# thanh-nt25/Whisper-context-biasing

Hardware: AMD Instinct MI355X
Metric: audio-seconds/sec (RTF) + biased-WER, whisper-small 30s clips, batch32 (higher is better)
Workload: dtype bf16

## Files before the change

### whisper_context_biasing_amd/csrc/k_logmel.hip

```cpp
#include <type_traits>

#include "common.h"
#include "kernels.h"

namespace wcb {

constexpr int kNFFT = 400, kHop = 160, kFrames = 3000, kNSamp = 480000;
constexpr int kFPB = 64;
constexpr int kSpan = (kFPB - 1) * kHop + 416;
constexpr int kNCol = 416;
constexpr int kBins = 201;

WCB_DEV unsigned ord_enc(float f) {
  const unsigned u = __float_as_uint(f);
  return (u & 0x80000000u) ? ~u : (u | 0x80000000u);
}
WCB_DEV float ord_dec(unsigned u) { return __uint_as_float((u & 0x80000000u) ? (u & 0x7fffffffu) : ~u); }

struct MelFixed {};
struct MelLong { int n_total, T, T_ld; const int* n_valid; };
template <bool SPLIT, bool LONG = false>
__global__ __launch_bounds__(256) void logmel_power_mel_kernel(const float* __restrict__ pcm, long pcm_stride, int n_valid,
                                                               const float* __restrict__ dft, const uint16_t* __restrict__ dft3,
                                                               const int* __restrict__ mel_lo,
                                                               const int* __restrict__ mel_hi, const float* __restrict__ mel_w,
                                                               int n_mel, float* __restrict__ out, unsigned* __restrict__ clip_max,
                                                               [[maybe_unused]] std::conditional_t<LONG, MelLong, MelFixed> shape) {
  constexpr int kPowLd = kBins + 3;
  constexpr int kLdsFloats = (kSpan > kFPB * kPowLd) ? kSpan : kFPB * kPowLd;
  __shared__ __attribute__((aligned(16))) float lds[kLdsFloats];
  __shared__ float wmax[4];
  const int b = blockIdx.y, f0 = blockIdx.x * kFPB;
  const int tid = threadIdx.x, lane = tid & 63, wave = tid >> 6;
  const float* x = pcm + (long)b * pcm_stride;
  int nS = kNSamp, nF = kFrames, ldo = kFrames;
  if constexpr (LONG) { nS = shape.n_total; nF = shape.T; ldo = shape.T_ld; n_valid = shape.n_valid[b]; }
// ... 75 lines not shown
  }
  }
  __syncthreads();
#pragma unroll
  for (int i = 0; i < 4; ++i)
#pragma unroll
    for (int j = 0; j < kCW; ++j)
#pragma unroll
      for (int e = 0; e < 4; ++e) {
        const float v = acc[i][j][e];
        const float p = v * v + __shfl_xor(v, 1, 64) * __shfl_xor(v, 1, 64);
        const int col = (cf0 + j) * 16 + (lane & 15);
        if (j < ncf && (col & 1) == 0 && (col >> 1) < kBins)
          lds[(i * 16 + (lane >> 4) * 4 + e) * kPowLd + (col >> 1)] = p;
      }
  __syncthreads();
  float lmax = -INFINITY;
  for (int idx = tid; idx < n_mel * kFPB; idx += 256) {
    const int m = idx / kFPB, f = idx % kFPB;
    if (f0 + f >= nF) continue;
    const int lo = mel_lo[m], hi = mel_hi[m];
    float s = 0.f;
    for (int k = lo; k < hi; ++k) s = fmaf(mel_w[m * 32 + (k - lo)], lds[f * kPowLd + k], s);
    const float lg = log10f(fmaxf(s, 1e-10f));
    out[((long)b * n_mel + m) * ldo + f0 + f] = lg;
    lmax = fmaxf(lmax, lg);
  }
  lmax = wave_max(lmax);
  if (lane == 0) wmax[wave] = lmax;
  __syncthreads();
  if (tid == 0) atomicMax(clip_max + b, ord_enc(fmaxf(fmaxf(wmax[0], wmax[1]), fmaxf(wmax[2], wmax[3]))));
}

__global__ void logmel_normalize_kernel(float* mel, const unsigned* clip_max, int n_per_clip, long total) {
  for (long i = blockIdx.x * (long)blockDim.x + threadIdx.x; i < total; i += (long)gridDim.x * blockDim.x) {
    const float mx = ord_dec(clip_max[i / n_per_clip]);
    mel[i] = (fmaxf(mel[i], mx - 8.0f) + 4.0f) / 4.0f;
  }
}

__global__ void logmel_normalize_long_kernel(float* mel, const unsigned* clip_max, int n_mel, int T, int T_ld, long total) {
  for (long i = blockIdx.x * (long)blockDim.x + threadIdx.x; i < total; i += (long)gridDim.x * blockDim.x) {
    const long row = i / T;
    const float mx = ord_dec(clip_max[row / n_mel]);
    float* p = mel + row * T_ld + (i - row * T);
    *p = (fmaxf(*p, mx - 8.0f) + 4.0f) / 4.0f;
  }
}

void logmel_power_mel(const float* pcm, long pcm_stride, int n_samples, int B, const float* dft, const void* dft3,
                      const int* mel_lo, const int* mel_hi, const float* mel_w, int n_mel, float* mel_out,
                      unsigned* clip_max, hipStream_t s) {
  (void)hipMemsetAsync(clip_max, 0, sizeof(unsigned) * B, s);
  const dim3 grid((kFrames + kFPB - 1) / kFPB, B);
  if (dft3)
    WCB_LAUNCH(logmel_power_mel_kernel<true>, grid, dim3(256), 0, s, pcm, pcm_stride, n_samples, dft,
               reinterpret_cast<const uint16_t*>(dft3), mel_lo, mel_hi, mel_w, n_mel, mel_out, clip_max, MelFixed{});
  else
    WCB_LAUNCH(logmel_power_mel_kernel<false>, grid, dim3(256), 0, s, pcm, pcm_stride, n_samples, dft,
               nullptr, mel_lo, mel_hi, mel_w, n_mel, mel_out, clip_max, MelFixed{});
}

void logmel_long(const float* pcm, long pcm_stride, const int* n_valid, int n_total, int B, const float* dft, const void* dft3,
                 const int* mel_lo, const int* mel_hi, const float* mel_w, int n_mel, float* mel_out, int T_ld,
                 unsigned* clip_max, hipStream_t s) {
  const int T = n_total / kHop;
  (void)hipMemsetAsync(clip_max, 0, sizeof(unsigned) * B, s);
  const dim3 grid((T + kFPB - 1) / kFPB, B);
  const MelLong shape{n_total, T, T_ld, n_valid};
  if (dft3)
    WCB_LAUNCH((logmel_power_mel_kernel<true, true>), grid, dim3(256), 0, s, pcm, pcm_stride, 0, dft,
               reinterpret_cast<const uint16_t*>(dft3), mel_lo, mel_hi, mel_w, n_mel, mel_out, clip_max, shape);
  else
    WCB_LAUNCH((logmel_power_mel_kernel<false, true>), grid, dim3(256), 0, s, pcm, pcm_stride, 0, dft,
               nullptr, mel_lo, mel_hi, mel_w, n_mel, mel_out, clip_max, shape);
  const long total = (long)B * n_mel * T;
  WCB_LAUNCH(logmel_normalize_long_kernel, dim3(2048), dim3(256), 0, s, mel_out, clip_max, n_mel, T, T_ld, total);
}

void logmel_normalize(float* mel, const unsigned* clip_max, int B, int n_mel, hipStream_t s) {
  const long total = (long)B * n_mel * kFrames;
  WCB_LAUNCH(logmel_normalize_kernel, dim3(2048), dim3(256), 0, s, mel, clip_max, n_mel * kFrames, total);
}

template <typename T>
__global__ void mel_to_conv_input_kernel(const float* __restrict__ mel, int n_mel, T* __restrict__ xt, long clip_stride) {
  __shared__ float tile[64][65];
  const int b = blockIdx.z, t0 = blockIdx.x * 64, c0 = blockIdx.y * 64;
  for (int i = threadIdx.x; i < 64 * 64; i += 256) {
    const int c = c0 + i / 64, t = t0 + i % 64;
    tile[i / 64][i % 64] = (c < n_mel && t < kFrames) ? mel[((long)b * n_mel + c) * kFrames + t] : 0.f;
  }
  __syncthreads();
  for (int i = threadIdx.x; i < 64 * 64; i += 256) {
    const int t = t0 + i / 64, c = c0 + i % 64;
    if (t < kFrames && c < n_mel) xt[(long)b * clip_stride + (long)(t + 1) * n_mel + c] = DT<T>::fromf(tile[i % 64][i / 64]);
  }
  if (blockIdx.x == 0 && blockIdx.y == 0)
    for (int c = threadIdx.x; c < n_mel; c += 256) {
      xt[(long)b * clip_stride + c] = DT<T>::fromf(0.f);
      xt[(long)b * clip_stride + (long)(kFrames + 1) * n_mel + c] = DT<T>::fromf(0.f);
    }
}
// ... 46 lines not shown
```

### whisper_context_biasing_amd/csrc/kernels.h

```cpp
#pragma once
#include <hip/hip_runtime.h>
#include <hip/hip_ext.h>
#include <stdint.h>

#include "tsrule.h"

namespace wcb {

struct LaunchTimer {
  hipEvent_t start = nullptr, stop = nullptr;
  int n = 0;
  const void* fn = nullptr;
  long grid = 0;
};
inline thread_local LaunchTimer g_launch_timer;

#define WCB_LAUNCH(K, G, B, SH, S, ...)                                                              \
  do {                                                                                               \
    ::wcb::LaunchTimer& lt_ = ::wcb::g_launch_timer;                                                 \
    if (lt_.stop) {                                                                                  \
      if (!lt_.n) {                                                                                  \
        lt_.fn = reinterpret_cast<const void*>(K);                                                   \
        const dim3 g_ = dim3(G), b_ = dim3(B);                                                       \
        lt_.grid = (long)g_.x * g_.y * g_.z * b_.x * b_.y * b_.z;                                    \
// ... 97 lines not shown
  const int* phys = nullptr; long phys_ld = 0;
  int causal = 0;
  int q_log2 = 0;
  int xcd_nqb = 0;
  int kv_rows = 0;
  const int* key_start = nullptr;
};
void attention_decode(DType t, const AttnArgs& a, hipStream_t s);
bool attention_flash(DType t, const AttnArgs& a, hipStream_t s);

constexpr int kXencMaxSplit = 16;
struct XencArgs {
  const void* enc = nullptr; long enc_sb = 0;
  const void* qp = nullptr;
  int rows = 0, H = 0, D = 0, S = 0;
  int nsplit = 1;
  float* part = nullptr;
  float* ml = nullptr;
  Stamp stamp;
  int variant = 1;
  int row0 = 0, rows_per_enc = 1;
  int fm = 0;
  int part16 = 0;
  int merge_os = 1;
};
bool xenc_supported(DType t, int D);
void xenc_to_fm(DType t, const void* src, void* dst, int B, int S, int D, hipStream_t s);
long xenc_fm_elems(int B, int S, int D);
void xenc_attention(DType t, const XencArgs& a, hipStream_t s);
void xenc_merge(DType t, const XencArgs& a, void* u, long ldu, hipStream_t s);
void xenc_merge_v(DType t, const XencArgs& a, const void* wv, const float* bv, void* o, long ldo, hipStream_t s,
                  const void* wv_fm = nullptr);

void logmel_power_mel(const float* pcm, long pcm_stride, int n_samples, int B, const float* dft, const void* dft3,
                      const int* mel_lo, const int* mel_hi, const float* mel_w, int n_mel,
                      float* mel_out, unsigned* clip_max, hipStream_t s);
void logmel_normalize(float* mel, const unsigned* clip_max, int B, int n_mel, hipStream_t s);
void mel_to_conv_input(DType t, const float* mel, int B, int n_mel, void* xt, long clip_stride,
                       hipStream_t s);
void logmel_long(const float* pcm, long pcm_stride, const int* n_valid, int n_total, int B, const float* dft, const void* dft3,
                 const int* mel_lo, const int* mel_hi, const float* mel_w, int n_mel, float* mel_out, int T_ld,
                 unsigned* clip_max, hipStream_t s);
void mel_window_to_conv_input(DType t, const float* mel, int n_mel, int T_ld, const int* clip_idx, const int* seek, const int* nfr,
                              int rows, void* xt, long row_stride, hipStream_t s);

struct ForestArgs {
  const int* root = nullptr;
  const int* rc_off = nullptr;
  const int* rc_tok = nullptr;
  const int* rc_dst = nullptr;
};
void forest_init(const ForestArgs& f, int* state, int* rowbase, int R, int nb, hipStream_t s);

struct SelectArgs {
  const float* logits = nullptr; long ld = 0; int M = 0; int V = 0;
  float lam = 0.f; const uint32_t* root_bits = nullptr;
  const int* trans_off = nullptr; const int* trans_tok = nullptr; const int* trans_dst = nullptr;
  const int* root_child = nullptr;
  const int* st_depth = nullptr; const int* st_keep = nullptr;
  int* state = nullptr; int* finished = nullptr;
  int* rowbase = nullptr;
  int eos = 0, pad = 0; int min_new = 0;
  int* step = nullptr;
  int* pos = nullptr;
  int* next_ids = nullptr; int* out_ids = nullptr; int out_ld = 0;
  float* part_val = nullptr; int* part_idx = nullptr; int nchunk = 0;
  int* all_done = nullptr;
  unsigned long long* ticket_unfin = nullptr;
  float* out_score = nullptr;
  const float* part_max = nullptr; const float* part_sum = nullptr;
  float* out_logprob = nullptr;
  const void* emb = nullptr; const void* pemb = nullptr; int n_pos = 0, d = 0, dtype = 0;
  float* x = nullptr; void* x16 = nullptr; void* x16fm = nullptr; int fm_nw = 0, fm_kpw = 0;
// ... 134 lines not shown
```

### whisper_context_biasing_amd/csrc/runtime.cpp

```cpp
#include <hip/hip_runtime.h>

#include <algorithm>
#include <cxxabi.h>
#include <cmath>
#include <cstdio>
#include <cstring>
#include <map>
#include <thread>
#include <memory>
#include <stdexcept>
#include <string>
#include <vector>
#include <cstdlib>
#include <deque>
#include <atomic>

#include "../../include/wcb.h"
#include "kernels.h"
#include "sample.h"
#include "dtw.h"

using namespace wcb;

namespace {
// ... 165 lines not shown
};

struct wcb_handle {
  wcb_model_desc d{};
  DType dt = kBF16;
  int device = 0;
  std::string err;
  hipStream_t he = nullptr;
  static constexpr int kMaxCtx = 4;
  int nctx = 2;
  hipEvent_t ev_xkv[kMaxCtx] = {}, ev_dec[kMaxCtx] = {};
  int gen_count = 0;
  hipEvent_t ev_in = nullptr, ev_out = nullptr;
  static constexpr int kMaxSub = DecCtx::kMaxSub;
  DecCtx dc[kMaxCtx];
  int n_sub = 1;
  int xsplit = 1;
  int xvariant = 0;
  int flash_split = 2;
  int beam_xattn = 0;
  int ln_fold = 1;
  int merge_v = 1;
  int xpart16 = 1;
  int xq_kq = 0;
  int ring_kt = 2;
  int beam_wide = 1;
  int beam_wfm = 0;
  int lean_fold = 1;
  int xqk = 1;
  int xqk_nch = 8;
  int merge_os = 1;
  int lm_walkers = 256;
  int mel_split = 0;
  int lean_mf2 = 0;
  int beam_chunks = 0;
  int beam_raster = 0;
  int lm_ln_split = 0;
  int enc_flash_qw = 4;
  int xmode = 1;
  int beam_xmode = 0;
  int group_rows = 512;
  int xenc_split = 6;
  int xenc_fm = 1;
  int xenc_variant = 1;
  int ln16 = 1;
  int vocab_pad = 0;
  int steps_per_graph = 8;
  int lean = 1;
  int lean_x = 1;
  int64_t n_graph_captures = 0;
  struct wcb_state* step_state = nullptr;
  bool rules_on = false, rules_has0 = false;
  TsRule rules_ts;
  DevBuf rules_deny, rules_deny0;
  int enc_raster = 8;
  int enc_gemm = 4;
  bool dec_gemm = false;
  std::map<std::string, DevBuf> staged;
  std::vector<DevBuf> owned;
  bool ready = false;
  int dbg_enc_layers = -1;
  void *conv1_w = nullptr, *conv2_w = nullptr;
  float *conv1_b = nullptr, *conv2_b = nullptr, *enc_pos = nullptr;
  int k1pad = 0;
  std::vector<LayerW> enc, dec;
  float *enc_ln_w = nullptr, *enc_ln_b = nullptr, *dec_ln_w = nullptr, *dec_ln_b = nullptr;
  void* xkv_w = nullptr; float* xkv_b = nullptr;
  void *tok_emb = nullptr, *dec_pos = nullptr;
  void* tok_emb_fm = nullptr;
  DevBuf dft, dft3, mel_lo, mel_hi, mel_w, clip_max;
  DevBuf win_ints;
  int enc_B = 0;
  DevBuf xt, hbuf, x, h, qkv, att, ffn, encout;
  DevBuf xkv2[kMaxCtx];
  DevBuf al_w, al_M, al_tf, al_lens, al_frames, al_prefix, al_trace;
  int last_gen_buf = -1, last_gen_B = 0, last_gen_xm = 0, last_gen_id = -1;
  hipEvent_t ev_align = nullptr;
  bool align_pending = false;
  size_t align_ws_bytes = (size_t)1 << 30;
  std::unique_ptr<wcb_bias> empty_bias;
  std::vector<wcb_bias*> biases;
  DevBuf dev_err;
  bool prof = false, prof_stamps = false;
  std::vector<ProfEntry> prof_e;
  std::deque<std::pair<int, std::pair<hipEvent_t, hipEvent_t>>> prof_pending;
  std::vector<hipEvent_t> ev_pool;
  DevBuf stamps, stamp_acc;
  static constexpr int kStampRegions = 8;
  unsigned long long* stamp_base(int buf, int region) {
    return stamps.as<unsigned long long>() + ((size_t)buf * kStampRegions + region) * stamp_slots() * 2 * kStampSub;
  }
  double xattn_bytes = 0, xattn_flops = 0;
  long stamp_slots() const { return (long)d.n_text_ctx * d.n_layers * kMaxSub; }

  int H() const { return d.n_heads; }
  int S() const { return d.n_audio_ctx; }

  void* upload(const void* src, size_t bytes) {
    owned.emplace_back();
    owned.back().ensure(bytes);
    HIPCHK(hipMemcpy(owned.back().p, src, bytes, hipMemcpyHostToDevice));
    return owned.back().p;
  }
// ... 87 lines not shown
    f();
    return WCB_OK;
  } catch (const WcbError& e) {
    (h ? h->err : g_err) = e.what();
    return e.code;
  } catch (const std::exception& e) {
    (h ? h->err : g_err) = e.what();
    return WCB_ERR_ARG;
  }
}

double hz_to_mel(double f) { return f >= 1000.0 ? 15.0 + std::log(f / 1000.0) * (27.0 / std::log(6.4)) : 3.0 * f / 200.0; }
double mel_to_hz(double m) { return m >= 15.0 ? 1000.0 * std::exp((std::log(6.4) / 27.0) * (m - 15.0)) : 200.0 * m / 3.0; }

std::vector<double> mel_filters(int n_mel) {
  const int nf = 201;
  std::vector<double> mf(n_mel + 2), ff(n_mel + 2), fft(nf), out((size_t)nf * n_mel, 0.0);
  const double mmin = hz_to_mel(0.0), mmax = hz_to_mel(8000.0);
  for (int i = 0; i < n_mel + 2; ++i) {
    mf[i] = (i == n_mel + 1) ? mmax : mmin + i * ((mmax - mmin) / (n_mel + 1));
    ff[i] = mel_to_hz(mf[i]);
  }
  for (int k = 0; k < nf; ++k) fft[k] = (k == nf - 1) ? 8000.0 : k * (8000.0 / (nf - 1));
  for (int k = 0; k < nf; ++k)
    for (int m = 0; m < n_mel; ++m) {
      const double down = -(ff[m] - fft[k]) / (ff[m + 1] - ff[m]);
      const double up = (ff[m + 2] - fft[k]) / (ff[m + 2] - ff[m + 1]);
      const double v = std::max(0.0, std::min(down, up));
      out[(size_t)k * n_mel + m] = v * (2.0 / (ff[m + 2] - ff[m]));
    }
  return out;
}

}

extern "C" {

const char* wcb_last_error(const wcb_handle* h) { return h ? h->err.c_str() : g_err.c_str(); }

int wcb_create(const wcb_model_desc* desc, int device, wcb_handle** out) {
  return guarded(nullptr, [&] {
    REQUIRE(desc && out, "null argument");
    REQUIRE(desc->d_model % 64 == 0 && desc->d_model / desc->n_heads == 64, "head_dim must be 64");
    REQUIRE(desc->dtype >= 0 && desc->dtype <= 2, "dtype");
    REQUIRE(desc->n_mel == 80 || desc->n_mel == 128, "n_mel must be 80 or 128");
    REQUIRE(desc->n_audio_ctx * 2 == kFrames, "n_audio_ctx must be 1500");
    HIPCHK(hipSetDevice(device));
    auto h = std::make_unique<wcb_handle>();
    h->d = *desc;
    h->dt = DType(desc->dtype);
    h->device = device;
    HIPCHK(hipStreamCreateWithPriority(&h->he, hipStreamNonBlocking, 0));
    for (int ci = 0; ci < wcb_handle::kMaxCtx; ++ci) {
      DecCtx& D = h->dc[ci];
      HIPCHK(hipEventCreateWithFlags(&D.ev_fork, hipEventDisableTiming));
      HIPCHK(hipHostMalloc(reinterpret_cast<void**>(&D.done_h), 2 * sizeof(int), hipHostMallocDefault));
      for (hipEvent_t& e : D.ev_poll) HIPCHK(hipEventCreateWithFlags(&e, hipEventDisableTiming));
      for (int i = 0; i < DecCtx::kMaxSub; ++i) HIPCHK(hipEventCreateWithFlags(&D.ev_join[i], hipEventDisableTiming));
    }
    for (int i = 0; i < wcb_handle::kMaxCtx; ++i) {
      HIPCHK(hipEventCreateWithFlags(&h->ev_xkv[i], hipEventDisableTiming));
      HIPCHK(hipEventCreateWithFlags(&h->ev_dec[i], hipEventDisableTiming));
    }
    HIPCHK(hipEventCreateWithFlags(&h->ev_in, hipEventDisableTiming));
    HIPCHK(hipEventCreateWithFlags(&h->ev_out, hipEventDisableTiming));
    h->xvariant = desc->n_heads >= 20 ? 1 : 0;
    h->xmode = xenc_supported(h->dt, desc->d_model) ? 1 : 0;
    h->beam_xmode = 0;
    if (h->dt == kF32) h->ln16 = 0;
    h->dec_gemm = gemm_dec_supported(h->dt, desc->d_model);
    std::vector<float> dft((size_t)kNCol * kNCol, 0.f);
    for (int c = 0; c < 402; ++c) {
      const int bin = c >> 1;
      for (int k = 0; k < 400; ++k) {
        const double win = 0.5 - 0.5 * std::cos(2.0 * M_PI * k / 400.0);
        const double ang = 2.0 * M_PI * (double)((long)bin * k % 400) / 400.0;
        dft[(size_t)c * kNCol + k] = (float)(win * ((c & 1) ? -std::sin(ang) : std::cos(ang)));
      }
    }
    h->dft.ensure(dft.size() * 4);
    HIPCHK(hipMemcpy(h->dft.p, dft.data(), dft.size() * 4, hipMemcpyHostToDevice));
    {
      auto bf = [](double v, double& back) -> uint16_t {
        const float f = (float)v;
        uint32_t u;
        std::memcpy(&u, &f, 4);
        u += 0x7fffu + ((u >> 16) & 1u);
        const uint16_t hbits = (uint16_t)(u >> 16);
        const uint32_t w = (uint32_t)hbits << 16;
        float g;
        std::memcpy(&g, &w, 4);
        back = g;
        return hbits;
      };
      std::vector<uint16_t> t3((size_t)3 * kNCol * kNCol, 0);
      for (int c = 0; c < 402; ++c) {
        const int bin = c >> 1;
        for (int k = 0; k < 400; ++k) {
          const double win = 0.5 - 0.5 * std::cos(2.0 * M_PI * k / 400.0);
          const double ang = 2.0 * M_PI * (double)((long)bin * k % 400) / 400.0;
          double r = win * ((c & 1) ? -std::sin(ang) : std::cos(ang)), back;
          for (int part = 0; part < 3; ++part) {
            t3[(size_t)part * kNCol * kNCol + (size_t)c * kNCol + k] = bf(r, back);
            r -= back;
          }
        }
      }
      h->dft3.ensure(t3.size() * 2);
      HIPCHK(hipMemcpy(h->dft3.p, t3.data(), t3.size() * 2, hipMemcpyHostToDevice));
    }
    const auto fb = mel_filters(desc->n_mel);
    std::vector<int> lo(desc->n_mel), hi(desc->n_mel);
    std::vector<float> w((size_t)desc->n_mel * 32, 0.f);
    for (int m = 0; m < desc->n_mel; ++m) {
      int a = -1, b = -1;
      for (int k = 0; k < 201; ++k)
        if ((float)fb[(size_t)k * desc->n_mel + m] != 0.f) { if (a < 0) a = k; b = k; }
      if (a < 0) { a = 0; b = -1; }
      REQUIRE(b - a + 1 <= 32, "mel filter wider than 32 bins");
      lo[m] = a;
      hi[m] = b + 1;
      for (int k = a; k <= b; ++k) w[(size_t)m * 32 + (k - a)] = (float)fb[(size_t)k * desc->n_mel + m];
    }
    h->mel_lo.ensure(lo.size() * 4);
    h->mel_hi.ensure(hi.size() * 4);
    h->mel_w.ensure(w.size() * 4);
    HIPCHK(hipMemcpy(h->mel_lo.p, lo.data(), lo.size() * 4, hipMemcpyHostToDevice));
    HIPCHK(hipMemcpy(h->mel_hi.p, hi.data(), hi.size() * 4, hipMemcpyHostToDevice));
    HIPCHK(hipMemcpy(h->mel_w.p, w.data(), w.size() * 4, hipMemcpyHostToDevice));
    auto eb = std::make_unique<wcb_bias>();
    eb->vocab = desc->vocab;
    const int nw = (desc->vocab + 31) / 32;
    eb->root_bits.ensure((size_t)nw * 4);
    eb->root_child.ensure((size_t)desc->vocab * 4);
    HIPCHK(hipMemsetAsync(eb->root_child.p, 0xff, (size_t)desc->vocab * 4, nullptr));
    HIPCHK(hipStreamSynchronize(nullptr));
    std::vector<int> off = {0, 0};
    eb->trans_off.ensure(8);
    HIPCHK(hipMemcpy(eb->trans_off.p, off.data(), 8, hipMemcpyHostToDevice));
    eb->trans_tok.ensure(4);
    eb->trans_dst.ensure(4);
    eb->st_depth.ensure(4);
// ... 4 lines not shown
  });
}

void wcb_destroy(wcb_handle* h) {
  if (!h) return;
  (void)hipSetDevice(h->device);
  (void)hipDeviceSynchronize();
  for (wcb_bias* b : h->biases) b->owner = nullptr;
  for (DecCtx& D : h->dc) {
    D.drop_graphs();
    for (DevBuf* b : {&D.kvself, &D.dx, &D.dx16, &D.dx16fm, &D.dh, &D.dq, &D.dqp, &D.du, &D.datt, &D.dffn, &D.dstats, &D.drst, &D.xpart, &D.xml, &D.xticket,
                      &D.logits, &D.part_val, &D.part_idx, &D.ints, &D.outbuf, &D.forced, &D.beam, &D.kq_cnt, &D.part_max, &D.part_sum,
                      &D.lpbuf})
      b->release();
    if (D.ev_fork) (void)hipEventDestroy(D.ev_fork);
    for (hipEvent_t e : D.ev_poll)
      if (e) (void)hipEventDestroy(e);
    if (D.done_h) (void)hipHostFree(D.done_h);
    D.forest.release();
    D.poff.release();
    D.nsp.release();
    D.lang.release();
    if (D.p_stage) (void)hipHostFree(D.p_stage);
    if (D.ev_pcopy) (void)hipEventDestroy(D.ev_pcopy);
    if (D.f_stage) (void)hipHostFree(D.f_stage);
    if (D.ev_fcopy) (void)hipEventDestroy(D.ev_fcopy);
    for (int i = 0; i < DecCtx::kMaxSub; ++i) {
      if (D.ev_join[i]) (void)hipEventDestroy(D.ev_join[i]);
      if (D.sub[i]) (void)hipStreamDestroy(D.sub[i]);
    }
    if (D.hs) (void)hipStreamDestroy(D.hs);
  }
  for (auto& b : h->owned) b.release();
  for (DevBuf* b : {&h->dft, &h->dft3, &h->mel_lo, &h->mel_hi, &h->mel_w, &h->clip_max, &h->win_ints, &h->xt, &h->hbuf, &h->x, &h->h,
                    &h->qkv, &h->att, &h->ffn, &h->encout, &h->stamps, &h->stamp_acc, &h->dev_err, &h->rules_deny,
                    &h->rules_deny0, &h->al_w, &h->al_M, &h->al_tf, &h->al_lens, &h->al_frames, &h->al_prefix, &h->al_trace})
    b->release();
  for (auto e : h->ev_pool) (void)hipEventDestroy(e);
  if (h->ev_align) (void)hipEventDestroy(h->ev_align);
  if (h->ev_in) (void)hipEventDestroy(h->ev_in);
  if (h->ev_out) (void)hipEventDestroy(h->ev_out);
  if (h->he) (void)hipStreamDestroy(h->he);
  for (int i = 0; i < wcb_handle::kMaxCtx; ++i) {
    h->xkv2[i].release();
    if (h->ev_xkv[i]) (void)hipEventDestroy(h->ev_xkv[i]);
    if (h->ev_dec[i]) (void)hipEventDestroy(h->ev_dec[i]);
  }
  delete h;
}

namespace {
void quiesce(wcb_handle* h);
void drop_graphs(wcb_handle* h);
}

int wcb_set_option(wcb_handle* h, const char* name, int value) {
  return guarded(h, [&] {
    REQUIRE(h && name, "bad argument");
    const std::string n = name;
    static const char* const kFreeWhileStepwise[] = {"decode_contexts", "enc_flash", "enc_gemm", "enc_raster",
                                                     "steps_per_graph", "kq_cnt_seed", "align_ws"};
    bool free_opt = false;
    for (const char* f : kFreeWhileStepwise) free_opt |= n == f;
    REQUIRE(free_opt || !h->step_state, "option " + n + ": a step-wise decode is active (wcb_decode_end first)");
    if (n == "xmode" || n == "beam_xmode") {
      REQUIRE(!h->ready, "option " + n + " selects the weight layouts: set it before wcb_finalize_weights");
      REQUIRE(value == 0 || value == 1, "option " + n + ": 0 or 1");
// ... 33 lines not shown
      }
    } else if (n == "align_ws") {
      REQUIRE(value >= 1 && value <= 65536, "option align_ws: 1..65536 (MiB)");
      h->align_ws_bytes = (size_t)value << 20;
    } else if (n == "steps_per_graph") {
      REQUIRE(value >= 1 && value <= 64, "option steps_per_graph: 1..64");
      h->steps_per_graph = value;
    } else if (n == "xenc_fm") {
      h->xenc_fm = value != 0;
    } else if (n == "xq_kq") {
      h->xq_kq = value != 0;
    } else if (n == "enc_gemm") {
      REQUIRE(value == 0 || value == 1 || value == 4 || value == 5, "option enc_gemm: 0, 1, 4 or 5");
      h->enc_gemm = value;
    } else if (n == "enc_raster") {
      REQUIRE(value >= 0 && value <= 64, "option enc_raster: 0..64");
      h->enc_raster = value;
    } else if (n == "lean") {
      REQUIRE(!h->ready, "option lean selects weight layouts: set it before wcb_finalize_weights");
      h->lean = value != 0;
    } else if (n == "lean_x") {
      h->lean_x = value != 0;
    } else if (n == "xpart16") {
      h->xpart16 = value != 0;
    } else if (n == "merge_v") {
      h->merge_v = value != 0;
    } else if (n == "ln_fold") {
      REQUIRE(!h->ready, "option ln_fold selects weight layouts: set it before wcb_finalize_weights");
      h->ln_fold = value != 0;
    } else if (n == "lean_mf2") {
      h->lean_mf2 = value != 0;
    } else if (n == "mel_split") {
      h->mel_split = value != 0;
    } else if (n == "lm_walkers") {
      REQUIRE(!h->ready, "option lm_walkers sizes the argmax partials: set it before wcb_finalize_weights");
      REQUIRE(value == 128 || value == 192 || value == 256 || value == 384 || value == 512 || value == 1024,
              "option lm_walkers: 128, 192, 256, 384, 512 or 1024");
      h->lm_walkers = value;
    } else if (n == "merge_os") {
      REQUIRE(value == 1 || value == 2, "option merge_os: 1 or 2");
      h->merge_os = value;
    } else if (n == "xqk_chunks") {
      REQUIRE(value == 2 || value == 4 || value == 8 || value == 16, "option xqk_chunks: 2, 4, 8 or 16");
      h->xqk_nch = value;
    } else if (n == "xqk") {
      h->xqk = value != 0;
    } else if (n == "lean_fold") {
      REQUIRE(!h->ready, "option lean_fold selects weight layouts: set it before wcb_finalize_weights");
      h->lean_fold = value != 0;
    } else if (n == "beam_chunks") {
      h->beam_chunks = value != 0;
    } else if (n == "beam_wfm") {
      REQUIRE(!h->ready, "option beam_wfm selects weight layouts: set it before wcb_finalize_weights");
      h->beam_wfm = value != 0;
    } else if (n == "beam_raster") {
      REQUIRE(value >= 0 && value <= 64, "option beam_raster: 0..64");
      h->beam_raster = value;
    } else if (n == "beam_wide") {
      REQUIRE(!h->ready, "option beam_wide selects weight layouts: set it before wcb_finalize_weights");
      h->beam_wide = value != 0;
    } else if (n == "beam_xattn") {
      REQUIRE(value >= 0 && value <= 3, "option beam_xattn: 0..3");
      h->beam_xattn = value;
    } else if (n == "flash_split") {
      REQUIRE(value >= 1 && value <= kXSplit, "option flash_split: 1..8");
      h->flash_split = value;
// ... 1218 lines not shown
  }
  g.key = key;
}

struct GenCall {
  const float* mel; int B; const wcb_gen_cfg* cfg;
  const int32_t* prefix; int prefix_len;
  int32_t *out_ids, *out_steps;
  void* stream;
  const wcb_bias* bias = nullptr; const wcb_bias_batch* bb = nullptr;
  float *out_logprobs = nullptr, *out_seq_scores = nullptr;
  const wcb_sample_cfg* smp = nullptr;
  const int32_t* prompts = nullptr; int prompt_ld = 0; const int32_t* prompt_len = nullptr;
  const wcb_windows* win = nullptr; float* out_no_speech = nullptr;
  const wcb_lang_cfg* lang = nullptr;
};

DecCtx& step_ctx(wcb_handle* h, const wcb_state* st, bool what = true, const char* msg = "bad argument (state of this handle)") {
  REQUIRE(h && st && st->h == h && h->step_state == st && what, msg);
  return h->dc[wcb_handle::kMaxCtx - 1];
}

}

extern "C" {

int wcb_log_mel(wcb_handle* h, const float* pcm, int B, int n_samples, int64_t pcm_stride, float* mel_out, void* stream) {
  return guarded(h, [&] {
    REQUIRE(h && pcm && mel_out && B > 0 && n_samples > 0, "bad argument");
    REQUIRE(pcm_stride >= std::min(n_samples, kNSamp), "pcm_stride < n_samples");
    if ((size_t)B * 4 > h->clip_max.bytes) { quiesce(h); h->clip_max.ensure((size_t)std::max(B, h->enc_B) * 4); }
    sync_in(h, stream, h->he);
    h->timed("log_mel", 0, (double)B * (std::min(n_samples, kNSamp) * 4.0 + h->d.n_mel * kFrames * 4.0 * 3), h->he, [&] {
      logmel_power_mel(pcm, (long)pcm_stride, n_samples, B, h->dft.as<float>(), h->mel_split ? h->dft3.p : nullptr,
                       h->mel_lo.as<int>(), h->mel_hi.as<int>(),
                       h->mel_w.as<float>(), h->d.n_mel, mel_out, h->clip_max.as<unsigned>(), h->he);
      logmel_normalize(mel_out, h->clip_max.as<unsigned>(), B, h->d.n_mel, h->he);
    });
    sync_out(h, stream, h->he);
  });
}

int wcb_encode(wcb_handle* h, const float* mel, int B, void* enc_out, void* stream) {
  return guarded(h, [&] {
    REQUIRE(h && mel && B > 0, "bad argument");
    if (!h->ready) throw WcbError(WCB_ERR_STATE, "weights not finalized");
    ensure_enc_ws(h, B);
    sync_in(h, stream, h->he);
    encode_impl(h, mel, B, enc_out);
    sync_out(h, stream, h->he);
  });
}

int wcb_log_mel_long(wcb_handle* h, const float* pcm, int B, const int32_t* n_valid, int n_total, int64_t pcm_stride,
                     float* mel_out, int T_ld, void* stream) {
  return guarded(h, [&] {
    REQUIRE(h && pcm && mel_out && n_valid && B > 0 && B <= kWinRows, "bad argument (1 .. 64 clips)");
    REQUIRE(n_total >= 800 && pcm_stride >= n_total, "n_total must be at least 800 samples and at most pcm_stride");
    REQUIRE(T_ld >= n_total / 160, "T_ld < n_total / 160 frames");
    for (int b = 0; b < B; ++b) REQUIRE(n_valid[b] >= 0 && n_valid[b] <= n_total, "n_valid outside [0, n_total]");
    if ((size_t)B * 4 > h->clip_max.bytes) { quiesce(h); h->clip_max.ensure((size_t)std::max(B, h->enc_B) * 4); }
    h->win_ints.ensure((size_t)3 * kWinRows * 4);
    sync_in(h, stream, h->he);
    write_i32(h->win_ints.as<int>(), n_valid, B, h->he);
    h->timed("log_mel_long", 0, (double)B * (n_total * 4.0 + h->d.n_mel * (n_total / 160) * 4.0 * 3), h->he, [&] {
      logmel_long(pcm, (long)pcm_stride, h->win_ints.as<int>(), n_total, B, h->dft.as<float>(), h->mel_split ? h->dft3.p : nullptr,
                  h->mel_lo.as<int>(), h->mel_hi.as<int>(), h->mel_w.as<float>(), h->d.n_mel, mel_out, T_ld,
                  h->clip_max.as<unsigned>(), h->he);
    });
    sync_out(h, stream, h->he);
  });
}

int wcb_encode_windows(wcb_handle* h, const wcb_windows* w, int rows, void* enc_out, void* stream) {
  return guarded(h, [&] {
    REQUIRE(h, "bad argument");
    check_windows(w, rows);
    if (!h->ready) throw WcbError(WCB_ERR_STATE, "weights not finalized");
    ensure_enc_ws(h, rows);
    sync_in(h, stream, h->he);
    encode_impl(h, nullptr, rows, enc_out, w);
    sync_out(h, stream, h->he);
  });
}

static void generate_impl(wcb_handle* h, const GenCall& c) {
  {
    const wcb_gen_cfg* cfg = c.cfg;
    const wcb_sample_cfg* smp = c.smp;
    const wcb_bias_batch* bb = c.bb;
    const int B = c.B;
    REQUIRE(h && cfg && c.out_ids && c.out_steps && B > 0, "bad argument");
    if (!h->ready) throw WcbError(WCB_ERR_STATE, "weights not finalized");
    const int nb = cfg->num_beams;
    REQUIRE(nb >= 1 && nb <= kMaxBeams, "num_beams must be in [1, 8]");
    if (smp) {
      check_sampling(smp->temperature, smp->seeds);
      if (nb > 1) throw WcbError(WCB_ERR_UNSUPPORTED, "sampling is greedy only (num_beams = 1)");
    }
    if (h->rules_on && nb > 1)
// ... 1622 lines not shown
```

Measured before the change: 20090.

## Replace dense DFT log-mel with in-LDS mixed-radix real FFT

Adds a log-mel kernel that computes the 400-point STFT as a 200-point complex FFT (radix 5x5x8) in double precision in shared memory, with a real-FFT split, replacing the dense DFT matrix multiply. It becomes the default path, and the old DFT tables are now uploaded only when the option is switched off. This is meant to cut the arithmetic and the DFT-table memory traffic of the front end, but it brings fp64 math and small 8-frame blocks with several barriers. Log-mel is a small part of end-to-end Whisper throughput.

```diff
diff --git a/whisper_context_biasing_amd/csrc/k_logmel.hip b/whisper_context_biasing_amd/csrc/k_logmel.hip
--- a/whisper_context_biasing_amd/csrc/k_logmel.hip
+++ b/whisper_context_biasing_amd/csrc/k_logmel.hip
@@ -2,6 +2,7 @@
 
 #include "common.h"
 #include "kernels.h"
+#include "logmel_fft.h"
 
 namespace wcb {
 
@@ -143,6 +144,83 @@
   if (tid == 0) atomicMax(clip_max + b, ord_enc(fmaxf(fmaxf(wmax[0], wmax[1]), fmaxf(wmax[2], wmax[3]))));
 }
 
+constexpr int kFftFrames = 8;
+using MelF = MelFft<kFftFrames>;
+template <bool LONG>
+__global__ __launch_bounds__(MelF::kThreads) void logmel_fft_kernel(const float* __restrict__ pcm, long pcm_stride, int n_valid,
+                                                                    const cd* __restrict__ w400, const float* __restrict__ win,
+                                                                    const int* __restrict__ mel_lo, const int* __restrict__ mel_hi,
+                                                                    const float* __restrict__ mel_w, int n_mel,
+                                                                    float* __restrict__ out, unsigned* __restrict__ clip_max,
+                                                                    [[maybe_unused]] std::conditional_t<LONG, MelLong, MelFixed> shape) {
+  constexpr int kT = MelF::kThreads, kFF = kFftFrames, kPowLd = MelF::kPowLd;
+  constexpr int kSpFloats = MelF::kSpan > kFF * kPowLd ? MelF::kSpan : kFF * kPowLd;
+  __shared__ cd z[kFF * MelF::kZLd];
+  __shared__ __attribute__((aligned(16))) float sp[kSpFloats];
+  __shared__ float wmax[kT / 64];
+  static_assert(sizeof(cd) * kFF * MelF::kZLd + 4 * kSpFloats + 4 * (kT / 64) <= 64 * 1024, "at most 64 KiB of LDS");
+  static_assert(kT % 64 == 0, "whole waves");
+  const int b = blockIdx.y, f0 = blockIdx.x * kFF;
+  const int tid = threadIdx.x, lane = tid & 63, wave = tid >> 6;
+  const float* x = pcm + (long)b * pcm_stride;
+  int nS = kNSamp, nF = kFrames, ldo = kFrames;
+  if constexpr (LONG) { nS = shape.n_total; nF = shape.T; ldo = shape.T_ld; n_valid = shape.n_valid[b]; }
+  const int nv = min(n_valid, nS);
+  const int s0 = f0 * kHop - kNFFT / 2;
+  constexpr int kStageRounds = (MelF::kSpan + kT - 1) / kT;
+  float sv[kStageRounds];
+#pragma unroll
+  for (int it = 0; it < kStageRounds; ++it) {
+    int j = s0 + tid + it * kT;
+    if (j < 0) j = -j;
+    if (j >= nS) j = 2 * (nS - 1) - j;
+    j = max(0, min(j, nS - 1));
+    sv[it] = (tid + it * kT < MelF::kSpan && j < nv) ? x[j] : 0.f;
+  }
+#pragma unroll
+  for (int it = 0; it < kStageRounds; ++it)
+    if (tid + it * kT < MelF::kSpan) sp[tid + it * kT] = sv[it];
+  __syncthreads();
+  MelF::pass_a(tid, sp, win, z);
+  __syncthreads();
+  cd v[5];
+  MelF::pass_b_load(tid, z, w400, v);
+  __syncthreads();
+  MelF::pass_b_store(tid, z, v);
+  __syncthreads();
+  MelF::pass_c(tid, z, w400);
+  __syncthreads();
+  MelF::power(tid, z, w400, sp);
+  __syncthreads();
+  float lmax = -INFINITY;
+  for (int idx = tid; idx < n_mel * kFF; idx += kT) {
+    const int m = idx / kFF, f = idx % kFF;
+    if (f0 + f >= nF) continue;
+    const int lo = mel_lo[m], hi = mel_hi[m];
+    const float4* wrow = reinterpret_cast<const float4*>(mel_w + m * 32);
+    const float* prow = sp + f * kPowLd;
+    float s = 0.f;
+    for (int k = lo; k < hi; k += 8) {
+      const float4 w0 = wrow[(k - lo) >> 2], w1 = wrow[((k - lo) >> 2) + 1];
+      const float w[8] = {w0.x, w0.y, w0.z, w0.w, w1.x, w1.y, w1.z, w1.w};
+#pragma unroll
+      for (int e = 0; e < 8; ++e) s = fmaf(w[e], k + e < hi ? prow[k + e] : 0.f, s);
+    }
+    const float lg = log10f(fmaxf(s, 1e-10f));
+    out[((long)b * n_mel + m) * ldo + f0 + f] = lg;
+    lmax = fmaxf(lmax, lg);
+  }
+  lmax = wave_max(lmax);
+  if (lane == 0) wmax[wave] = lmax;
+  __syncthreads();
+  if (tid == 0) {
+    float mx = wmax[0];
+#pragma unroll
+    for (int w = 1; w < kT / 64; ++w) mx = fmaxf(mx, wmax[w]);
+    atomicMax(clip_max + b, ord_enc(mx));
+  }
+}
+
 __global__ void logmel_normalize_kernel(float* mel, const unsigned* clip_max, int n_per_clip, long total) {
   for (long i = blockIdx.x * (long)blockDim.x + threadIdx.x; i < total; i += (long)gridDim.x * blockDim.x) {
     const float mx = ord_dec(clip_max[i / n_per_clip]);
@@ -159,10 +237,18 @@
   }
 }
 
-void logmel_power_mel(const float* pcm, long pcm_stride, int n_samples, int B, const float* dft, const void* dft3,
+void logmel_power_mel(const float* pcm, long pcm_stride, int n_samples, int B, const MelTables& t,
                       const int* mel_lo, const int* mel_hi, const float* mel_w, int n_mel, float* mel_out,
                       unsigned* clip_max, hipStream_t s) {
   (void)hipMemsetAsync(clip_max, 0, sizeof(unsigned) * B, s);
+  if (t.w400) {
+    WCB_LAUNCH(logmel_fft_kernel<false>, dim3((kFrames + kFftFrames - 1) / kFftFrames, B), dim3(MelF::kThreads), 0, s, pcm,
+               pcm_stride, n_samples, reinterpret_cast<const cd*>(t.w400), t.win, mel_lo, mel_hi, mel_w, n_mel, mel_out, clip_max,
+               MelFixed{});
+    return;
+  }
+  const float* dft = t.dft;
+  const void* dft3 = t.dft3;
   const dim3 grid((kFrames + kFPB - 1) / kFPB, B);
   if (dft3)
     WCB_LAUNCH(logmel_power_mel_kernel<true>, grid, dim3(256), 0, s, pcm, pcm_stride, n_samples, dft,
@@ -172,14 +258,19 @@
                nullptr, mel_lo, mel_hi, mel_w, n_mel, mel_out, clip_max, MelFixed{});
 }
 
-void logmel_long(const float* pcm, long pcm_stride, const int* n_valid, int n_total, int B, const float* dft, const void* dft3,
+void logmel_long(const float* pcm, long pcm_stride, const int* n_valid, int n_total, int B, const MelTables& t,
                  const int* mel_lo, const int* mel_hi, const float* mel_w, int n_mel, float* mel_out, int T_ld,
                  unsigned* clip_max, hipStream_t s) {
   const int T = n_total / kHop;
   (void)hipMemsetAsync(clip_max, 0, sizeof(unsigned) * B, s);
   const dim3 grid((T + kFPB - 1) / kFPB, B);
   const MelLong shape{n_total, T, T_ld, n_valid};
-  if (dft3)
+  const float* dft = t.dft;
+  const void* dft3 = t.dft3;
+  if (t.w400)
+    WCB_LAUNCH(logmel_fft_kernel<true>, dim3((T + kFftFrames - 1) / kFftFrames, B), dim3(MelF::kThreads), 0, s, pcm, pcm_stride, 0,
+               reinterpret_cast<const cd*>(t.w400), t.win, mel_lo, mel_hi, mel_w, n_mel, mel_out, clip_max, shape);
+  else if (dft3)
     WCB_LAUNCH((logmel_power_mel_kernel<true, true>), grid, dim3(256), 0, s, pcm, pcm_stride, 0, dft,
                reinterpret_cast<const uint16_t*>(dft3), mel_lo, mel_hi, mel_w, n_mel, mel_out, clip_max, shape);
   else
diff --git a/whisper_context_biasing_amd/csrc/kernels.h b/whisper_context_biasing_amd/csrc/kernels.h
--- a/whisper_context_biasing_amd/csrc/kernels.h
+++ b/whisper_context_biasing_amd/csrc/kernels.h
@@ -153,13 +153,14 @@
 void xenc_merge_v(DType t, const XencArgs& a, const void* wv, const float* bv, void* o, long ldo, hipStream_t s,
                   const void* wv_fm = nullptr);
 
-void logmel_power_mel(const float* pcm, long pcm_stride, int n_samples, int B, const float* dft, const void* dft3,
+struct MelTables { const void* w400; const float* win; const float* dft; const void* dft3; };
+void logmel_power_mel(const float* pcm, long pcm_stride, int n_samples, int B, const MelTables& t,
                       const int* mel_lo, const int* mel_hi, const float* mel_w, int n_mel,
                       float* mel_out, unsigned* clip_max, hipStream_t s);
 void logmel_normalize(float* mel, const unsigned* clip_max, int B, int n_mel, hipStream_t s);
 void mel_to_conv_input(DType t, const float* mel, int B, int n_mel, void* xt, long clip_stride,
                        hipStream_t s);
-void logmel_long(const float* pcm, long pcm_stride, const int* n_valid, int n_total, int B, const float* dft, const void* dft3,
+void logmel_long(const float* pcm, long pcm_stride, const int* n_valid, int n_total, int B, const MelTables& t,
                  const int* mel_lo, const int* mel_hi, const float* mel_w, int n_mel, float* mel_out, int T_ld,
                  unsigned* clip_max, hipStream_t s);
 void mel_window_to_conv_input(DType t, const float* mel, int n_mel, int T_ld, const int* clip_idx, const int* seek, const int* nfr,
diff --git a/whisper_context_biasing_amd/csrc/logmel_fft.h b/whisper_context_biasing_amd/csrc/logmel_fft.h
--- /dev/null
+++ b/whisper_context_biasing_amd/csrc/logmel_fft.h
@@ -0,0 +1,111 @@
+#pragma once
+
+#ifndef WCB_HD
+#define WCB_HD __host__ __device__ __forceinline__
+#endif
+
+namespace wcb {
+
+struct alignas(16) cd { double r, i; };
+
+WCB_HD cd cadd(cd a, cd b) { return cd{a.r + b.r, a.i + b.i}; }
+WCB_HD cd csub(cd a, cd b) { return cd{a.r - b.r, a.i - b.i}; }
+WCB_HD cd cmul(cd a, cd b) { return cd{a.r * b.r - a.i * b.i, a.r * b.i + a.i * b.r}; }
+WCB_HD cd cmul_mi(cd a) { return cd{a.i, -a.r}; }
+
+WCB_HD void bfly5(cd* v) {
+  constexpr double c1 = 0.30901699437494742410, c2 = -0.80901699437494742410;
+  constexpr double s1 = 0.95105651629515357212, s2 = 0.58778525229247312917;
+  const cd t1 = cadd(v[1], v[4]), t2 = cadd(v[2], v[3]), t3 = csub(v[1], v[4]), t4 = csub(v[2], v[3]);
+  const cd a1{v[0].r + c1 * t1.r + c2 * t2.r, v[0].i + c1 * t1.i + c2 * t2.i};
+  const cd a2{v[0].r + c2 * t1.r + c1 * t2.r, v[0].i + c2 * t1.i + c1 * t2.i};
+  const cd b1{s1 * t3.r + s2 * t4.r, s1 * t3.i + s2 * t4.i};
+  const cd b2{s2 * t3.r - s1 * t4.r, s2 * t3.i - s1 * t4.i};
+  v[0] = cd{v[0].r + t1.r + t2.r, v[0].i + t1.i + t2.i};
+  v[1] = cd{a1.r + b1.i, a1.i - b1.r};
+  v[4] = cd{a1.r - b1.i, a1.i + b1.r};
+  v[2] = cd{a2.r + b2.i, a2.i - b2.r};
+  v[3] = cd{a2.r - b2.i, a2.i + b2.r};
+}
+
+WCB_HD constexpr int rev8(int r) { return ((r & 1) << 2) | (r & 2) | (r >> 2); }
+WCB_HD void bfly8(cd* v) {
+  constexpr double h = 0.70710678118654752440;
+#define WCB_FFT2(a, b) { const cd t = v[a]; v[a] = cadd(t, v[b]); v[b] = csub(t, v[b]); }
+  WCB_FFT2(0, 4) WCB_FFT2(1, 5) WCB_FFT2(2, 6) WCB_FFT2(3, 7)
+  v[5] = cd{h * (v[5].r + v[5].i), h * (v[5].i - v[5].r)};
+  v[6] = cmul_mi(v[6]);
+  v[7] = cd{h * (v[7].i - v[7].r), -h * (v[7].r + v[7].i)};
+  WCB_FFT2(0, 2) WCB_FFT2(1, 3) WCB_FFT2(4, 6) WCB_FFT2(5, 7)
+  v[3] = cmul_mi(v[3]);
+  v[7] = cmul_mi(v[7]);
+  WCB_FFT2(0, 1) WCB_FFT2(2, 3) WCB_FFT2(4, 5) WCB_FFT2(6, 7)
+#undef WCB_FFT2
+}
+
+template <int FF>
+struct MelFft {
+  static constexpr int kHop = 160, kN = 400, kM = 200, kBins = 201;
+  static constexpr int kThreads = 40 * FF;
+  static constexpr int kSpan = (FF - 1) * kHop + kN;
+  static constexpr int kZLd = kM + 1;
+  static constexpr int kPowLd = kBins;
+
+  WCB_HD static void pass_a(int tid, const float* sp, const float* win, cd* z) {
+    const int f = tid / 40, j = tid % 40;
+    cd v[5];
+#pragma unroll
+    for (int r = 0; r < 5; ++r) {
+      const int n = 2 * (j + 40 * r);
+      const float a = sp[f * kHop + n] * win[n], b = sp[f * kHop + n + 1] * win[n + 1];
+      v[r] = cd{(double)a, (double)b};
+    }
+    bfly5(v);
+#pragma unroll
+    for (int r = 0; r < 5; ++r) z[f * kZLd + 5 * j + r] = v[r];
+  }
+
+  WCB_HD static void pass_b_load(int tid, const cd* z, const cd* w400, cd* v) {
+    const int f = tid / 40, j = tid % 40, k = j % 5;
+    v[0] = z[f * kZLd + j];
+#pragma unroll
+    for (int r = 1; r < 5; ++r) v[r] = cmul(z[f * kZLd + j + 40 * r], w400[16 * r * k]);
+    bfly5(v);
+  }
+  WCB_HD static void pass_b_store(int tid, cd* z, const cd* v) {
+    const int f = tid / 40, j = tid % 40;
+    const int j0 = (j / 5) * 25 + j % 5;
+#pragma unroll
+    for (int r = 0; r < 5; ++r) z[f * kZLd + j0 + 5 * r] = v[r];
+  }
+
+  WCB_HD static void pass_c(int tid, cd* z, const cd* w400) {
+    if (tid >= FF * 25) return;
+    const int f = tid / 25, j = tid % 25;
+    cd v[8];
+    v[0] = z[f * kZLd + j];
+#pragma unroll
+    for (int r = 1; r < 8; ++r) v[r] = cmul(z[f * kZLd + j + 25 * r], w400[2 * r * j]);
+    bfly8(v);
+#pragma unroll
+    for (int r = 0; r < 8; ++r) z[f * kZLd + j + 25 * rev8(r)] = v[r];
+  }
+
+  WCB_HD static void power(int tid, const cd* z, const cd* w400, float* pw) {
+    const int f = tid / 40, j = tid % 40;
+    cd w[5];
+#pragma unroll
+    for (int it = 0; it < 5; ++it) w[it] = w400[j + 40 * it];
+#pragma unroll
+    for (int it = 0; it < 5; ++it) {
+      const int k = j + 40 * it;
+      const cd a = z[f * kZLd + k], b = z[f * kZLd + (k ? kM - k : 0)];
+      const cd e{0.5 * (a.r + b.r), 0.5 * (a.i - b.i)}, o{0.5 * (a.i + b.i), 0.5 * (b.r - a.r)};
+      const cd x = cadd(e, cmul(w[it], o));
+      pw[f * kPowLd + k] = (float)(x.r * x.r + x.i * x.i);
+      if (k == 0) pw[f * kPowLd + kM] = (float)((a.r - a.i) * (a.r - a.i));
+    }
+  }
+};
+
+}
diff --git a/whisper_context_biasing_amd/csrc/runtime.cpp b/whisper_context_biasing_amd/csrc/runtime.cpp
--- a/whisper_context_biasing_amd/csrc/runtime.cpp
+++ b/whisper_context_biasing_amd/csrc/runtime.cpp
@@ -221,6 +221,7 @@
   int merge_os = 1;
   int lm_walkers = 256;
   int mel_split = 0;
+  int mel_fft = 1;
   int lean_mf2 = 0;
   int beam_chunks = 0;
   int beam_raster = 0;
@@ -257,7 +258,11 @@
   void* xkv_w = nullptr; float* xkv_b = nullptr;
   void *tok_emb = nullptr, *dec_pos = nullptr;
   void* tok_emb_fm = nullptr;
-  DevBuf dft, dft3, mel_lo, mel_hi, mel_w, clip_max;
+  DevBuf dft, dft3, fft_tab, mel_lo, mel_hi, mel_w, clip_max;
+  MelTables mel_tables() const {
+    if (mel_fft) return MelTables{fft_tab.p, reinterpret_cast<const float*>(static_cast<const char*>(fft_tab.p) + 400 * 16), nullptr, nullptr};
+    return MelTables{nullptr, nullptr, dft.as<float>(), mel_split ? dft3.p : nullptr};
+  }
   DevBuf win_ints;
   int enc_B = 0;
   DevBuf xt, hbuf, x, h, qkv, att, ffn, encout;
@@ -411,6 +416,50 @@
   return out;
 }
 
+void upload_dft_tables(wcb_handle* h) {
+  if (h->dft.p) return;
+  std::vector<float> dft((size_t)kNCol * kNCol, 0.f);
+  for (int c = 0; c < 402; ++c) {
+    const int bin = c >> 1;
+    for (int k = 0; k < 400; ++k) {
+      const double win = 0.5 - 0.5 * std::cos(2.0 * M_PI * k / 400.0);
+      const double ang = 2.0 * M_PI * (double)((long)bin * k % 400) / 400.0;
+      dft[(size_t)c * kNCol + k] = (float)(win * ((c & 1) ? -std::sin(ang) : std::cos(ang)));
+    }
+  }
+  h->dft.ensure(dft.size() * 4);
+  HIPCHK(hipMemcpy(h->dft.p, dft.data(), dft.size() * 4, hipMemcpyHostToDevice));
+  {
+    auto bf = [](double v, double& back) -> uint16_t {
+      const float f = (float)v;
+      uint32_t u;
+      std::memcpy(&u, &f, 4);
+      u += 0x7fffu + ((u >> 16) & 1u);
+      const uint16_t hbits = (uint16_t)(u >> 16);
+      const uint32_t w = (uint32_t)hbits << 16;
+      float g;
+      std::memcpy(&g, &w, 4);
+      back = g;
+      return hbits;
+    };
+    std::vector<uint16_t> t3((size_t)3 * kNCol * kNCol, 0);
+    for (int c = 0; c < 402; ++c) {
+      const int bin = c >> 1;
+      for (int k = 0; k < 400; ++k) {
+        const double win = 0.5 - 0.5 * std::cos(2.0 * M_PI * k / 400.0);
+        const double ang = 2.0 * M_PI * (double)((long)bin * k % 400) / 400.0;
+        double r = win * ((c & 1) ? -std::sin(ang) : std::cos(ang)), back;
+        for (int part = 0; part < 3; ++part) {
+          t3[(size_t)part * kNCol * kNCol + (size_t)c * kNCol + k] = bf(r, back);
+          r -= back;
+        }
+      }
+    }
+    h->dft3.ensure(t3.size() * 2);
+    HIPCHK(hipMemcpy(h->dft3.p, t3.data(), t3.size() * 2, hipMemcpyHostToDevice));
+  }
+}
+
 }
 
 extern "C" {
@@ -448,45 +497,17 @@
     h->beam_xmode = 0;
     if (h->dt == kF32) h->ln16 = 0;
     h->dec_gemm = gemm_dec_supported(h->dt, desc->d_model);
-    std::vector<float> dft((size_t)kNCol * kNCol, 0.f);
-    for (int c = 0; c < 402; ++c) {
-      const int bin = c >> 1;
+    {
+      std::vector<double> w(2 * 400);
+      std::vector<float> win(400);
       for (int k = 0; k < 400; ++k) {
-        const double win = 0.5 - 0.5 * std::cos(2.0 * M_PI * k / 400.0);
-        const double ang = 2.0 * M_PI * (double)((long)bin * k % 400) / 400.0;
-        dft[(size_t)c * kNCol + k] = (float)(win * ((c & 1) ? -std::sin(ang) : std::cos(ang)));
+        w[2 * k] = std::cos(2.0 * M_PI * k / 400.0);
+        w[2 * k + 1] = -std::sin(2.0 * M_PI * k / 400.0);
+        win[k] = (float)(0.5 - 0.5 * std::cos(2.0 * M_PI * k / 400.0));
       }
-    }
-    h->dft.ensure(dft.size() * 4);
-    HIPCHK(hipMemcpy(h->dft.p, dft.data(), dft.size() * 4, hipMemcpyHostToDevice));
-    {
-      auto bf = [](double v, double& back) -> uint16_t {
-        const float f = (float)v;
-        uint32_t u;
-        std::memcpy(&u, &f, 4);
-        u += 0x7fffu + ((u >> 16) & 1u);
-        const uint16_t hbits = (uint16_t)(u >> 16);
-        const uint32_t w = (uint32_t)hbits << 16;
-        float g;
-        std::memcpy(&g, &w, 4);
-        back = g;
-        return hbits;
-      };
-      std::vector<uint16_t> t3((size_t)3 * kNCol * kNCol, 0);
-      for (int c = 0; c < 402; ++c) {
-        const int bin = c >> 1;
-        for (int k = 0; k < 400; ++k) {
-          const double win = 0.5 - 0.5 * std::cos(2.0 * M_PI * k / 400.0);
-          const double ang = 2.0 * M_PI * (double)((long)bin * k % 400) / 400.0;
-          double r = win * ((c & 1) ? -std::sin(ang) : std::cos(ang)), back;
-          for (int part = 0; part < 3; ++part) {
-            t3[(size_t)part * kNCol * kNCol + (size_t)c * kNCol + k] = bf(r, back);
-            r -= back;
-          }
-        }
-      }
-      h->dft3.ensure(t3.size() * 2);
-      HIPCHK(hipMemcpy(h->dft3.p, t3.data(), t3.size() * 2, hipMemcpyHostToDevice));
+      h->fft_tab.ensure(w.size() * 8 + win.size() * 4);
+      HIPCHK(hipMemcpy(h->fft_tab.p, w.data(), w.size() * 8, hipMemcpyHostToDevice));
+      HIPCHK(hipMemcpy(static_cast<char*>(h->fft_tab.p) + w.size() * 8, win.data(), win.size() * 4, hipMemcpyHostToDevice));
     }
     const auto fb = mel_filters(desc->n_mel);
     std::vector<int> lo(desc->n_mel), hi(desc->n_mel);
@@ -557,7 +578,7 @@
     if (D.hs) (void)hipStreamDestroy(D.hs);
   }
   for (auto& b : h->owned) b.release();
-  for (DevBuf* b : {&h->dft, &h->dft3, &h->mel_lo, &h->mel_hi, &h->mel_w, &h->clip_max, &h->win_ints, &h->xt, &h->hbuf, &h->x, &h->h,
+  for (DevBuf* b : {&h->dft, &h->dft3, &h->fft_tab, &h->mel_lo, &h->mel_hi, &h->mel_w, &h->clip_max, &h->win_ints, &h->xt, &h->hbuf, &h->x, &h->h,
                     &h->qkv, &h->att, &h->ffn, &h->encout, &h->stamps, &h->stamp_acc, &h->dev_err, &h->rules_deny,
                     &h->rules_deny0, &h->al_w, &h->al_M, &h->al_tf, &h->al_lens, &h->al_frames, &h->al_prefix, &h->al_trace})
     b->release();
@@ -657,6 +678,12 @@
       h->lean_mf2 = value != 0;
     } else if (n == "mel_split") {
       h->mel_split = value != 0;
+    } else if (n == "mel_fft") {
+      if (value == 0) {
+        HIPCHK(hipSetDevice(h->device));
+        upload_dft_tables(h);
+      }
+      h->mel_fft = value != 0;
     } else if (n == "lm_walkers") {
       REQUIRE(!h->ready, "option lm_walkers sizes the argmax partials: set it before wcb_finalize_weights");
       REQUIRE(value == 128 || value == 192 || value == 256 || value == 384 || value == 512 || value == 1024,
@@ -1941,8 +1968,7 @@
     if ((size_t)B * 4 > h->clip_max.bytes) { quiesce(h); h->clip_max.ensure((size_t)std::max(B, h->enc_B) * 4); }
     sync_in(h, stream, h->he);
     h->timed("log_mel", 0, (double)B * (std::min(n_samples, kNSamp) * 4.0 + h->d.n_mel * kFrames * 4.0 * 3), h->he, [&] {
-      logmel_power_mel(pcm, (long)pcm_stride, n_samples, B, h->dft.as<float>(), h->mel_split ? h->dft3.p : nullptr,
-                       h->mel_lo.as<int>(), h->mel_hi.as<int>(),
+      logmel_power_mel(pcm, (long)pcm_stride, n_samples, B, h->mel_tables(), h->mel_lo.as<int>(), h->mel_hi.as<int>(),
                        h->mel_w.as<float>(), h->d.n_mel, mel_out, h->clip_max.as<unsigned>(), h->he);
       logmel_normalize(mel_out, h->clip_max.as<unsigned>(), B, h->d.n_mel, h->he);
     });
@@ -1973,8 +1999,7 @@
     sync_in(h, stream, h->he);
     write_i32(h->win_ints.as<int>(), n_valid, B, h->he);
     h->timed("log_mel_long", 0, (double)B * (n_total * 4.0 + h->d.n_mel * (n_total / 160) * 4.0 * 3), h->he, [&] {
-      logmel_long(pcm, (long)pcm_stride, h->win_ints.as<int>(), n_total, B, h->dft.as<float>(), h->mel_split ? h->dft3.p : nullptr,
-                  h->mel_lo.as<int>(), h->mel_hi.as<int>(), h->mel_w.as<float>(), h->d.n_mel, mel_out, T_ld,
+      logmel_long(pcm, (long)pcm_stride, h->win_ints.as<int>(), n_total, B, h->mel_tables(), h->mel_lo.as<int>(), h->mel_hi.as<int>(), h->mel_w.as<float>(), h->d.n_mel, mel_out, T_ld,
                   h->clip_max.as<unsigned>(), h->he);
     });
     sync_out(h, stream, h->he);
```

New measurement: 20220, median of 6. No clear change (+0.6%).
